# NorESMhub/BLOM

Measured on AMD Instinct MI355X. Metric: simulated-days/sec, higher is better.
Workload: dtype f64; 1 GPU; channel 208x512x53 as 1 tile(s) of 208x512x53 along i, 1 tile per GPU, isopyc_bulkml/remap/geopotential/uc/enscon, ntr=3 (TKE, length-scale slot, ideal age: the reference default build), baclin=900s batrop=18s lstep=50; config 2's step (phy/mod_blom_step.F90:96-253: init_fluxes, tmsmt1, cmnfld2, difest_isobml [the whole routine: diffusivities estimated every step (NorESM defaults incl. rhsctp; the; physics=full, forcing=default, spinup_steps=0

## Files before the change

### blom_amd/csrc/api.hip

```cpp
#include "../../include/blomgpu.h"
#include "blomgpu_internal.h"
#include "pow_libm.h"
#include "sin_libm.h"
#include "atan2_libm.h"
#include <cstring>

static thread_local std::string g_err;

int ctx_fail(blomgpu_ctx *c, const std::string &msg) {
  if (c) c->err = msg;
  g_err = msg;
  return 1;
}

void ctx_drop_graphs(blomgpu_ctx *c) {
  for (auto &g : c->step_graph)
    if (g) { (void)hipGraphExecDestroy(g); g = nullptr; }
  c->steps_warm = 0;
}

void ctx_sync_view(blomgpu_ctx *c) {
  if (!c->dirty) return;
  ctx_drop_graphs(c);
  (void)hipMemcpyAsync(c->d, &c->h, sizeof(DevView), hipMemcpyHostToDevice, c->stream);
// ... 284 lines not shown
  if (s == "tau_decaying_hml") { c->tau_decaying_hml = v; return 0; }
  if (s == "lfmin") { c->lfmin = v; return 0; }
  if (s == "cl") { c->eddtra_cl = v; return 0; }
  if (s == "mstar") { c->mstar = v; return 0; }
  if (s == "nstar") { c->nstar = v; return 0; }
  if (s == "wpup_min") { c->wpup_min = v; return 0; }
  if (s == "mlbl_max_ratio") { c->mlbl_max_ratio = v; return 0; }
  if (s == "ale_stab_fac_limit") { c->ale_stab_fac_limit = v; return 0; }
  if (s == "ale_dpvar_fac") { c->ale_dpvar_fac = v; return 0; }
  if (s == "ale_smooth_diff_max") { c->ale_smooth_diff_max = v; return 0; }
  if (s == "ale_dpmin_interior") { c->ale_dpmin_interior = v * 9806.; return 0; }
  return ctx_fail(c, "blomgpu_set_real: unknown option " + s);
}

int blomgpu_get_real(blomgpu_ctx *c, const char *name, double *v) {
  Params &P = c->h.P;
  std::string s(name);
#define R(nm) if (s == #nm) { *v = P.nm; return 0; }
  R(baclin) R(batrop) R(delt1) R(dlt) R(pref) R(wbaro)
#undef R
  if (s == "area") { *v = c->area; return 0; }
  if (s == "bdml_logc") { *v = c->bdml_logc; return 0; }
  if (s == "barotp_block_mode") { *v = bt_block_mode(c); return 0; }
  if (s == "graph_steps") { *v = c->graph_steps; return 0; }
  if (s == "graph_failures") { *v = c->graph_failures; return 0; }
  if (s == "mxlayr_maxitr_entrain" || s == "mxlayr_maxitr_detrain") {
    *v = 0.;
    if (!c->err_dev) return 0;
    const int w = s == "mxlayr_maxitr_detrain" ? 5 : 6;
    int n = 0;
    HIPCHK(c, hipStreamSynchronize(c->stream));
    HIPCHK(c, hipMemcpy(&n, c->err_dev + w, sizeof(int), hipMemcpyDeviceToHost));
    HIPCHK(c, hipMemset(c->err_dev + w, 0, sizeof(int)));
    *v = n;
    return 0;
  }
  return ctx_fail(c, "blomgpu_get_real: unknown option " + s);
}

int blomgpu_set_int(blomgpu_ctx *c, const char *name, int v) {
  std::string s(name);
  if (c && s == "timing") { c->timing = v != 0; return 0; }
  if (c) ctx_drop_graphs(c);
  Params &P = c->h.P;
#define R(nm) if (s == #nm) { P.nm = v; c->dirty = true; return 0; }
  if (s == "nstep") { P.nstep = v; return 0; }
// ... 676 lines not shown
```

### blom_amd/csrc/blomgpu_internal.h

```cpp
#pragma once
#include <hip/hip_runtime.h>
#include <cstdint>
#include <string>
#include <unordered_map>
#include <vector>
#include "exp_libm.h"

#define NBDY 4

#ifdef BLOM_HOSTEMU
#define WAIT_VMCNT0() ((void)0)
#else
#define WAIT_VMCNT0() asm volatile("s_waitcnt vmcnt(0)" ::: "memory")
#endif

#define BLOM_REAL_FIELDS(X)                                                              \
                                                                          \
  X(u, 2 * K) X(v, 2 * K) X(dp, 2 * K) X(dpu, 2 * K) X(dpv, 2 * K) X(temp, 2 * K)        \
  X(saln, 2 * K) X(sigma, 2 * K) X(uflx, 2 * K) X(vflx, 2 * K) X(utflx, 2 * K)           \
  X(vtflx, 2 * K) X(usflx, 2 * K) X(vsflx, 2 * K)                                        \
  X(p, K + 1) X(pu, K + 1) X(pv, K + 1) X(phi, K + 1) X(cau, K) X(cav, K)                \
  X(ubflxs, 3) X(vbflxs, 3) X(ub, 2) X(vb, 2) X(pb, 2) X(pbu, 2) X(pbv, 2)               \
  X(ubflxs_p, 2) X(vbflxs_p, 2) X(pb_p, 1) X(pbu_p, 1) X(pbv_p, 1) X(ubcors_p, 1)        \
  X(vbcors_p, 1) X(sealv, 1)                                                             \
// ... 206 lines not shown
  int tmsmt_fold = 1;
  bool pbcor1_handed_over = false;
  int steps_warm = 0;
  long long graph_steps = 0;
  int graph_failures = 0;
  int pgf_uv_pair = 0;
  int scan_reassoc = 0;
  hipStream_t side3 = nullptr;
  hipEvent_t ev_side3[2] = {nullptr, nullptr};
  int mom_aw_split = 0;
  int mom_aw_key = -1, mom_aw_n[2] = {0, 0};
  int *mom_aw_dev = nullptr;
  int mom_force_aw = 0;
  int convec_nsingle = 2;
  int cmn_nslope_nb = 4;
  int pgf_reuse = 0;
  int pgf_uv_ring = 7;
  int pgf_copy_fused = 1;
  int eddtra_frozen = 0;
  int check_period = 8;
  bool csdiag = false;
  bool bt_restart = true;
  unsigned bt_epoch = 0;
  int remap_fold = 0;
  int remap_nfirst = 4;
  bool remap_handed_over = false;
  int ale_method = 102, ale_upper_bndr_ord = 6, ale_lower_bndr_ord = 4, ale_tracer_limiting = 203, ale_velocity_limiting = 203;
  bool ale_tracer_pc_upper = true, ale_tracer_pc_lower = false, ale_velocity_pc_upper = true, ale_velocity_pc_lower = false;
  bool ale_density_pc_upper = false, ale_density_pc_lower = false;
  int ale_regrid_method = 2, ale_k_range_plevel = 1;
  double ale_regrid_nudge_ts = 86400., ale_stab_fac_limit = .75, ale_dpvar_fac = .75, ale_smooth_diff_max = 50000.;
  int ale_dktzu = 4, ale_dktzl = 2;
  double ale_dpmin_interior = .1 * 9806.;
  double rm0 = 1.2, rm5 = 0., niwgf = 0., niwbf = .35, niwlf = .5;
  std::string mlrttp = "constant";
  double trxday = 0., srxday = 0., trxdpt = 1., srxdpt = 1., trxlim = 1.5, srxlim = .5, sref = 34.65, area = 0., xmi = 0.;
  int lmi[5] = {11, 12, 1, 2, 3};
  bool aptflx = false, apsflx = false, ditflx = false, disflx = false, srxbal = false;
  int ntda = 0;
  bool full_physics = false;
  double swamxd = 200., brine_mlbase_frac = 0.;
  void *ale = nullptr;
  double *ale_plevel = nullptr;
  int mlrmth = 1;
  double eddtra_ce = .06, tau_mlr = 86400., tau_growing_hbl = 300., tau_decaying_hbl = 86400., tau_growing_hml = 3600.,
         tau_decaying_hml = 259200., lfmin = 5.e3, mlbl_max_ratio = 3., eddtra_cl = .25, mstar = .5, nstar = .066, wpup_min = 1.e-3;
  bool fluxes_lean = false;
// ... 107 lines not shown
int st_mxlayr_tail(blomgpu_ctx *, int nn, int k1n);
int ctx_err_words(blomgpu_ctx *);
int ctx_check_errors(blomgpu_ctx *);
int st_kfpla_halo(blomgpu_ctx *, int n);
int st_cmnfld1(blomgpu_ctx *, int m, int n, int mm, int nn, int k1m, int k1n);
int st_cmnfld2(blomgpu_ctx *, int m, int n, int mm, int nn, int k1m, int k1n);
int diapfl_column3_launch(blomgpu_ctx *, int n, int nn, int *errflag);
#define R_BASE(ntr) (8 + 3 * (ntr))
#define R_DP(ntr) (R_BASE(ntr) + 0)
#define R_T(ntr) (R_BASE(ntr) + 1)
#define R_S(ntr) (R_BASE(ntr) + 2)
#define R_TR(ntr, nt) (R_BASE(ntr) + 3 + (nt))
int st_ale_vdifft(blomgpu_ctx *, int m, int n, int mm, int nn, int k1m, int k1n);
int st_ale_vdiffm(blomgpu_ctx *, int m, int n, int mm, int nn, int k1m, int k1n);
int st_ale_forcing(blomgpu_ctx *, int m, int n, int mm, int nn, int k1m, int k1n);
int st_cmnfld_bfsqi_ale(blomgpu_ctx *, int m, int n, int mm, int nn, int k1m, int k1n);
int st_ale_regrid_remap(blomgpu_ctx *, int m, int n, int mm, int nn, int k1m, int k1n);
void ale_free(blomgpu_ctx *);
int ale_check_deferred(blomgpu_ctx *);
int st_mxlayr(blomgpu_ctx *, int m, int n, int mm, int nn, int k1m, int k1n);
int st_mom_pupv(blomgpu_ctx *, int off, int lo, int hi);
int st_convec_velocity(blomgpu_ctx *, int nn);
int launch_dpudpv(blomgpu_ctx *, int off, int flags);
int remap_tile_launch(blomgpu_ctx *, int n, int mm, int nn, int tsel, bool fold);
int pbcor_tile_launch(blomgpu_ctx *, int which, int m, int offc, int offf, int from_remap);
int launch_pscan(blomgpu_ctx *, int off, int lo, int hi_off);
int st_xctilr(blomgpu_ctx *, double *base, int l1, int ld, int mh, int nh, int itype);
int st_xctilr_arctic_multi(blomgpu_ctx *, int nf, double *const *ptrs, const int *nlevs, const int *mhs, const int *nhs,
                           const int *itypes);
int st_xctilr_multi(blomgpu_ctx *, int nf, double *const *ptrs, const int *nlevs, int mh, int nh, const int *itypes);
int st_crc(blomgpu_ctx *, const double *base, int nlev, int itype, unsigned *crc);
int st_crc_strips(blomgpu_ctx *, double *base, int nlev, int itype, unsigned *out, int cap, int *l0, int *ns);
int ctx_locate_ptr(const blomgpu_ctx *, const double *p, size_t *offset);
int rccl_xctilr(blomgpu_ctx *, double *base, int nlev, int mhl, int nhl);
int rccl_barotp_replicated(blomgpu_ctx *, int m, int n, int mm, int nn, int k1m, int k1n);
blomgpu_ctx *bt_global_ctx(const blomgpu_ctx *);
struct RcclLanded {
  const double *from_west = nullptr, *from_east = nullptr;
  int has_w = 0, has_e = 0, per = 0, mhl = 0, nhl = 0, nlev = 0;
  double *send_west = nullptr, *send_east = nullptr;
  int prepacked = 0;
};
int rccl_xctilr_multi_ex(blomgpu_ctx *, double *const *fields, int nf, int nlev, int mhl, int nhl, RcclLanded *landed);
int rccl_xctilr_multi(blomgpu_ctx *, double *const *fields, int nf, int nlev, int mhl, int nhl);

__device__ inline void xcd_block(unsigned &bx, unsigned &by) {
  const unsigned gx = gridDim.x, n = gx * gridDim.y;
// ... 26 lines not shown
```

### blom_amd/csrc/stage_advect.hip

```cpp
#include "remap_common.h"

#define THREAD_IJ(V)                                                       \
  unsigned bx_, by_;                                                       \
  xcd_block(bx_, by_);                                                     \
  const int t_ = bx_ * blockDim.x + threadIdx.x;                           \
  (void)by_;                                                               \
  if (t_ >= (V).nplane) return;                                            \
  const int i = t_ % (V).ni - (NBDY - 1), j = t_ / (V).ni - (NBDY - 1);    \
  const size_t c = t_

__global__ void k_adv_flux_area(const DevView *__restrict__ Vp, int m, int mm, int nn) {
  const DevView &V = *Vp;
  THREAD_IJ(V);
  if (j < 1 || j > V.jj || i < 1 || i > V.ii) return;
  const int k = by_;
  const size_t np = V.nplane, okm = c + (size_t)(k + mm) * np, okn = c + (size_t)(k + nn) * np;
  const size_t om = c + (size_t)(m - 1) * np;
  const double delt1 = V.P.delt1, dlt = V.P.dlt;
  if (V.m[I_iu][c]) {
    const double dtdl = delt1 * V.f[F_scuy][c];
    const double ca_tmp = V.f[F_u][okm] * dtdl + V.f[F_ubflxs_p][om] * dlt / V.f[F_pbu][om] +
                          (V.f[F_umfltd][okm] + V.f[F_umflsm][okm]) / fmax2(ONEMM, V.f[F_dpu][okn]);
    const double um = V.f[F_umax][c];
    V.f[F_cau][c + (size_t)k * np] = fmax2(-um * dtdl, fmin2(um * dtdl, ca_tmp));
// ... 104 lines not shown
    }
    if (int rc = st_xctilr(c, h.f[F_dp] + (size_t)(k1n - 1) * np, 1, h.kk, 1, 1, 1)) return rc;
    if (int rc = st_xctilr(c, h.f[F_temp] + (size_t)(k1n - 1) * np, 1, h.kk, 1, 1, 1)) return rc;
    if (int rc = st_xctilr(c, h.f[F_saln] + (size_t)(k1n - 1) * np, 1, h.kk, 1, 1, 1)) return rc;
    for (int nt = 0; nt < h.ntr; nt++)
      if (int rc = st_xctilr(c, h.f[F_trc] + ((size_t)(k1n - 1) + (size_t)nt * 2 * h.kk) * np, 1, h.kk, 1, 1, 1)) return rc;
    return 0;
  }
  hipLaunchKernelGGL(k_adv_pbmin, plane_grid(h), dim3(256), 0, c->stream, c->d);
  std::vector<double *> ptrs = {h.f[F_cau], h.f[F_cav]};
  std::vector<int> nl = {h.kk, h.kk}, it = {13, 14};
  for (int nt = 0; nt < h.ntr; nt++) {
    if (trc_skip_adv(h.P, nt + 1)) continue;
    ptrs.push_back(h.f[F_trc] + ((size_t)(k1n - 1) + (size_t)nt * 2 * h.kk) * np);
    nl.push_back(h.kk);
    it.push_back(1);
  }
  const int nf = (int)ptrs.size();
  auto halo_all = [&]() -> int {
    for (int f = 0; f < nf; f += 16)
      if (int rc = st_xctilr_multi(c, nf - f < 16 ? nf - f : 16, ptrs.data() + f, nl.data() + f, 3, 3, it.data() + f)) return rc;
    return 0;
  };
  const bool fold = c->in_sequence && c->remap_fold;
  const int mmlean = !fold && c->in_sequence && c->fluxes_zeroed && c->lean_fluxes ? mm : -1;
  const bool ovl = c->tiling.rccl && c->xstream && c->halo_overlap && !c->timing;
  if (ovl) {
    HIPCHK(c, hipEventRecord(c->ev_fork, c->stream));
    HIPCHK(c, hipStreamWaitEvent(c->xstream, c->ev_fork, 0));
    c->halo_stream = c->xstream;
    const int rc = halo_all();
    c->halo_stream = nullptr;
    if (rc) return rc;
    HIPCHK(c, hipEventRecord(c->ev_join, c->xstream));
    if (int rc2 = remap_tile_launch(c, n, mm, nn, 1, fold)) return rc2;
    HIPCHK(c, hipStreamWaitEvent(c->stream, c->ev_join, 0));
    if (int rc2 = remap_tile_launch(c, n, mm, nn, 2, fold)) return rc2;
    if (!fold) hipLaunchKernelGGL(k_remap_update, plane_grid(h, h.kk), dim3(256), 0, c->stream, c->d, nn, mmlean);
  } else {
    if (int rc = halo_all()) return rc;
    TimeScope ts(c, "remap");
    if (int rc = remap_tile_launch(c, n, mm, nn, 0, fold)) return rc;
    if (!fold) hipLaunchKernelGGL(k_remap_update, plane_grid(h, h.kk), dim3(256), 0, c->stream, c->d, nn, mmlean);
  }
  c->remap_handed_over = fold;
  HIPCHK(c, hipGetLastError());
  return 0;
}
```

### blom_amd/csrc/stage_remap_tile.hip

```cpp
#include "remap_common.h"

#ifndef RT_TH
#define RT_TH 8
#define RT_NT 512
#endif
#define RT_TW 32
#define RT_GW (RT_TW + 2)
#define RT_GN (RT_GW * (RT_TH + 2))
#define RT_SW (RT_TW + 4)
#define RT_SN (RT_SW * (RT_TH + 4))
#define RT_NB 4
#define RT_NSC(ntr) (4 + (ntr))
#define RT_NG(ntr) (10 + 3 * (ntr))
#define RT_G_DPT(ntr) (8 + 3 * (ntr))
#define RT_G_PUP(ntr) (9 + 3 * (ntr))

#define MP(m) ((m) & 1)
#define MU(m) (((m) >> 1) & 1)
#define MV(m) (((m) >> 2) & 1)

static_assert(RT_NT >= RT_SN && RT_NT == 2 * RT_TW * RT_TH, "thread count of k_remap_tile");

#ifdef BLOM_HOSTEMU
#define hmax8 max8
#define hmin8 min8
#define hmax2 fmax2
#define hmin2 fmin2
#else
#define hmax2 hw_max
#define hmin2 hw_min
__device__ inline double hw_max(double a, double b) { double r; asm("v_max_f64 %0, %1, %2" : "=v"(r) : "v"(a), "v"(b)); return r; }
__device__ inline double hw_min(double a, double b) { double r; asm("v_min_f64 %0, %1, %2" : "=v"(r) : "v"(a), "v"(b)); return r; }
__device__ inline double hmax8(double a, double b, double c, double d, double e, double f, double g, double h) {
  return hw_max(hw_max(hw_max(a, b), hw_max(c, d)), hw_max(hw_max(e, f), hw_max(g, h)));
// ... 38 lines not shown
struct AdvList {
  int idx[64];
};
template <bool MORE>
__device__ inline void add_contrib_t(const double *g, int ntr, int x, double pbface, double a, double ax, double ay, double axx,
                                     double ayy, double axy, Acc &A, PolyRec *rec, const int slot) {
  const double dpt = g[RT_G_DPT(ntr) * RT_GN + x];
  const double pup = g[RT_G_PUP(ntr) * RT_GN + x];
  const double dl = fmin2(dpt, fmax2(0., pbface - pup));
  const double dx = g[G_DX * RT_GN + x], dy = g[G_DY * RT_GN + x];
  const double fd = a * dl + ax * dx + ay * dy;
  A.fd = A.fd + fd;
  const double qx = ax * dl + axx * dx + axy * dy;
  const double qy = ay * dl + axy * dx + ayy * dy;
  A.ft = A.ft + fd * g[G_TD * RT_GN + x] + qx * g[G_TX * RT_GN + x] + qy * g[G_TY * RT_GN + x];
  A.fs = A.fs + fd * g[G_SD * RT_GN + x] + qx * g[G_SX * RT_GN + x] + qy * g[G_SY * RT_GN + x];
#pragma unroll
  for (int nt = 0; nt < MAXTR; nt++)
    if (nt < ntr)
      A.ftr[nt] = A.ftr[nt] + fd * g[G_TRD(nt) * RT_GN + x] + qx * g[G_TRX(nt) * RT_GN + x] + qy * g[G_TRY(nt) * RT_GN + x];
  if (MORE) { rec[slot].fd = fd; rec[slot].qx = qx; rec[slot].qy = qy; rec[slot].x = x; }
}

template <bool MORE, bool FOLD>
__global__ void __launch_bounds__(RT_NT, 4) k_remap_tile(const DevView *__restrict__ Vp, int n, int mm, int nn, int ntx, int nadv_all, int nfirst, AdvList L, int tsel KPROF_ARGS) {
  const DevView &V = *Vp;
  const int nadv = nfirst;
  const int base = 1;
  HIP_DYNAMIC_SHARED(double, lds)
  unsigned bx_, by_;
  xcd_block(bx_, by_);
  const int k = by_, ni = V.ni, nj = V.nj, ntr = V.ntr, t = threadIdx.x;
  constexpr int STX = FOLD ? RT_TW - 1 : RT_TW, STY = FOLD ? RT_TH - 1 : RT_TH;
  const int x0 = (bx_ % ntx) * STX, y0 = (bx_ / ntx) * STY;
  const bool zero_old = (tsel & 4) != 0;
  const bool lean = (tsel & 8) != 0;
  tsel &= 3;
  if (tsel) {
    const int jlast = V.jj + NBDY - 1 - ((V.nreg == 2 && V.j0 + V.jj == V.jtdm) ? 1 : 0);
    const bool inner = x0 - 2 >= NBDY && x0 + RT_TW + 1 <= V.ii + NBDY - 1 && y0 - 2 >= NBDY && y0 + RT_TH + 1 <= jlast;
    if (inner != (tsel == 1)) return;
  }
  const size_t np = V.nplane, ok = (size_t)k * np, okn = (size_t)(k + nn) * np, okm = (size_t)(k + mm) * np;
  [[maybe_unused]] const bool kp_on = t == 0 && k == 10;
  if (kp_on) KPROF_MARK(bx_, 0);
  double *const sc = lds;
  double *const gr = lds;
  double *const cuv = lds + RT_NG(nadv) * RT_GN;
  int *const mpl = (int *)(cuv + 2 * RT_GN);
  double *const m2s = (double *)(mpl + RT_SN);
  gci_t mpk = V.m[I_mpack];
  gcd_t scp2 = V.f[F_scp2], scp2i = V.f[F_scp2i];

  double sv[4 + MAXTR];
  int sm;
  size_t cs_keep = 0;
  {
    gcd_t f_dp = V.f[F_dp] + okn, f_p = V.f[F_p] + (size_t)(k + 1) * np, f_t = V.f[F_temp] + okn;
    gcd_t f_s = V.f[F_saln] + okn, f_tr = V.f[F_trc] + okn;
    const int xs = x0 - 2 + t % RT_SW, ys = y0 - 2 + t / RT_SW;
    const bool in = t < RT_SN && xs >= 0 && xs < ni && ys >= 0 && ys < nj;
    const size_t cs = in ? (size_t)ys * ni + xs : 0;
    sm = in ? mpk[cs] : 0;
    sv[0] = f_dp[cs]; sv[1] = f_p[cs]; sv[2] = f_t[cs]; sv[3] = f_s[cs];
#pragma unroll
    for (int a = 0; a < MAXTR; a++) sv[4 + a] = a < nadv ? f_tr[cs + (size_t)L.idx[a] * 2 * V.kk * np] : 0.;
    cs_keep = cs;
  }
  int gx, gy;
  if (t < RT_TW * RT_TH) { gx = t % RT_TW + 1; gy = t / RT_TW + 1; }
  else {
    const int r = t - RT_TW * RT_TH;
    if (r < RT_GW) { gx = r; gy = 0; }
// ... 11 lines not shown
    const bool inplane = gthread && x >= 0 && x < ni && y >= 0 && y < nj;
    const int i = x - (NBDY - 1), j = y - (NBDY - 1);
    const int xc = x < 1 ? 1 : (x > ni - 1 ? ni - 1 : x), yc = y < 1 ? 1 : (y > nj - 1 ? nj - 1 : y);
    const size_t c = (size_t)yc * ni + xc;
    cau_q = V.f[F_cau][c + ok];
    cav_q = V.f[F_cav][c + ok];
    s2_q = scp2[c];
    s2i_q = scp2i[c];
    pm = WK2(V, 0)[c];
    gpoint = inplane && j >= -1 && j <= V.jj + 2 && i >= -1 && i <= V.ii + 2;
  }
  const bool uface = t < RT_TW * RT_TH;
  const int ft = t % (RT_TW * RT_TH);
  const int fq = (ft / RT_TW + 1) * RT_GW + ft % RT_TW + 1;
  const int fx = x0 + ft % RT_TW, fy = y0 + ft / RT_TW;
  const bool fin = fx >= 1 && fx < ni - 1 && fy >= 1 && fy < nj - 1;
  const size_t fc = fin ? (size_t)fy * ni + fx : (size_t)ni + 1;
  const int fi = fx - (NBDY - 1), fj = fy - (NBDY - 1);
  const double caf = (uface ? V.f[F_cau] : V.f[F_cav])[fc + ok];
  const double pbf = (uface ? V.f[F_pbu] : V.f[F_pbv])[fc + (size_t)(n - 1) * np];
  gd_t const o_f = (uface ? V.f[F_uflx] : V.f[F_vflx]) + fc + okm;
  gd_t const o_ft = (uface ? V.f[F_utflx] : V.f[F_vtflx]) + fc + okm;
  gd_t const o_fs = (uface ? V.f[F_usflx] : V.f[F_vsflx]) + fc + okm;
  const bool own = !FOLD || (ft % RT_TW < RT_TW - 1 && ft / RT_TW < RT_TH - 1);
  const bool rd_old = uface && !zero_old && own;
  const double f_o = rd_old ? *o_f : 0., ft_o = rd_old ? *o_ft : 0., fs_o = rd_old ? *o_fs : 0.;

  if (t < RT_SN) {
    mpl[t] = sm;
#pragma unroll
    for (int s = 0; s < 4 + MAXTR; s++)
      if (s < 4 + nadv) sc[s * RT_SN + t] = sv[s];
  }
  if (gthread) { cuv[q] = cau_q; cuv[RT_GN + q] = cav_q; m2s[q] = s2_q; m2s[RT_GN + q] = s2i_q; }
  __syncthreads();
  if (kp_on) KPROF_MARK(bx_, 1);

  double gv[10 + 3 * MAXTR];
#pragma unroll
  for (int s = 0; s < 10 + 3 * MAXTR; s++) gv[s] = 0.;
  double cuc = 0., cvc = 0.;
  const int mpc = gthread ? mpl[sidx] : 0;
  gpoint = gpoint && MP(mpc);
  TNbr nb;
  nb.w = nb.e = nb.s = nb.n = nb.sw = nb.se = nb.nw = nb.ne = 0;
  double k_dxi = 0., k_dyi = 0., k_xd = 0., k_yd = 0.;
  if (gpoint) {
    const int a = MU(mpc), b = MU(mpl[sidx + 1]), d = MV(mpc), e = MV(mpl[sidx + RT_SW]);
    nb.w = sidx - a;
// ... 68 lines not shown
    for (int s = 0; s < 8 + 3 * MAXTR; s++)
      if (s < 8 + 3 * nadv) gr[s * RT_GN + q] = gv[s];
    gr[RT_G_DPT(nadv) * RT_GN + q] = gv[8 + 3 * MAXTR];
    gr[RT_G_PUP(nadv) * RT_GN + q] = gv[9 + 3 * MAXTR];
    cuv[q] = cuc;
    cuv[RT_GN + q] = cvc;
  }
  __syncthreads();
  if (kp_on) KPROF_MARK(bx_, 2);
  if (!MORE && !FOLD && !fin) return;

  const int mpf = fin ? mpl[(ft / RT_TW + 2) * RT_SW + ft % RT_TW + 2] : 0;
  const bool fmask = uface ? MU(mpf) : MV(mpf);
  const bool in_f = uface ? (fj >= 0 && fj <= V.jj + 1 && fi >= 0 && fi <= V.ii + 2) : (fj >= 0 && fj <= V.jj + 2 && fi >= 0 && fi <= V.ii + 1);
  if (!MORE && !FOLD && !in_f) return;
  const bool do_face = fin && in_f;
  PolyRec rec[3];
#pragma unroll
  for (int z = 0; z < 3; z++) { rec[z].fd = 0.; rec[z].qx = 0.; rec[z].qy = 0.; rec[z].x = fq; }
  Acc A;
  A.fd = 0.; A.ft = 0.; A.fs = 0.;
#pragma unroll
  for (int nt = 0; nt < MAXTR; nt++) A.ftr[nt] = 0.;
  if (do_face) {
  const int f_along = uface ? 1 : RT_GW, f_across = uface ? RT_GW : 1;
  const double cf = fmask ? (caf > 0. ? caf * m2s[RT_GN + fq - f_along] : caf * m2s[RT_GN + fq]) : 0.;
  if (fmask) {
    const double cuc0 = cuv[fq], cvc0 = cuv[RT_GN + fq];
    const bool near = cf > 0.;
    const double sh = near ? .5 : -.5;
    const int fb = near ? fq - f_along : fq;
    const double s2_c = m2s[fb], s2_m = m2s[fb - f_across], s2_p = m2s[fb + f_across];
    const double s2i_m = m2s[RT_GN + fb - f_across], s2i_p = m2s[RT_GN + fb + f_across];
    double a, ax, ay, axx, ayy, axy, x2, y2, x4, y4;
    if (uface) {
      const double cuc1 = cuv[fq + RT_GW], cvc1 = cuv[RT_GN + fq + RT_GW];
      const double ym = -.5 * (cvc0 + cvc1);
      const double xm = ((ym + .5) * cuc0 - (ym - .5) * cuc1 - 2. * cf) / (1. + cvc0 - cvc1);
      const int ic = near ? fq - 1 : fq;
      if (cvc0 > 0.) {
        const double xc0 = (xm * cvc0 - cuc0 * (ym + .5)) / (cvc0 + ym + .5);
        const double xc1 = xc0 * s2_c * s2i_m;
        x4 = xc0 + sh;
        y4 = -.5;
        triint(s2_m, xc1 + sh, .5, -cuc0 + sh, -cvc0 + .5, sh, .5, a, ax, ay, axx, ayy, axy);
        add_contrib_t<MORE>(gr, nadv, ic - RT_GW, pbf, a, ax, ay, axx, ayy, axy, A, rec, 0);
      } else {
        x4 = -cuc0 + sh;
        y4 = -cvc0 - .5;
      }
      if (cvc1 < 0.) {
        const double xc0 = (xm * cvc1 - cuc1 * (ym - .5)) / (cvc1 + ym - .5);
        const double xc1 = xc0 * s2_c * s2i_p;
        x2 = xc0 + sh;
        y2 = .5;
        triint(s2_p, xc1 + sh, -.5, sh, -.5, -cuc1 + sh, -cvc1 - .5, a, ax, ay, axx, ayy, axy);
        add_contrib_t<MORE>(gr, nadv, ic + RT_GW, pbf, a, ax, ay, axx, ayy, axy, A, rec, 1);
      } else {
        x2 = -cuc1 + sh;
        y2 = -cvc1 + .5;
      }
      penint(s2_c, sh, .5, x2, y2, xm + sh, ym, x4, y4, sh, -.5, a, ax, ay, axx, ayy, axy);
      add_contrib_t<MORE>(gr, nadv, ic, pbf, a, ax, ay, axx, ayy, axy, A, rec, 2);
      if (base && own) {
        *o_f = f_o + A.fd;
        *o_ft = ft_o + A.ft;
        *o_fs = fs_o + A.fs;
      }
    } else {
      const double cuc1 = cuv[fq + 1], cvc1 = cuv[RT_GN + fq + 1];
      const double xm = -.5 * (cuc0 + cuc1);
      const double ym = ((xm + .5) * cvc0 - (xm - .5) * cvc1 - 2. * cf) / (1. + cuc0 - cuc1);
      const int jc = near ? fq - RT_GW : fq;
      if (cuc0 > 0.) {
        const double yc0 = (ym * cuc0 - cvc0 * (xm + .5)) / (cuc0 + xm + .5);
        const double yc1 = yc0 * s2_c * s2i_m;
        x2 = -.5;
        y2 = yc0 + sh;
        triint(s2_m, .5, yc1 + sh, .5, sh, -cuc0 + .5, -cvc0 + sh, a, ax, ay, axx, ayy, axy);
        add_contrib_t<MORE>(gr, nadv, jc - 1, pbf, a, ax, ay, axx, ayy, axy, A, rec, 0);
      } else {
        x2 = -cuc0 - .5;
        y2 = -cvc0 + sh;
      }
      if (cuc1 < 0.) {
        const double yc0 = (ym * cuc1 - cvc1 * (xm - .5)) / (cuc1 + xm - .5);
        const double yc1 = yc0 * s2_c * s2i_p;
        x4 = .5;
        y4 = yc0 + sh;
        triint(s2_p, -.5, yc1 + sh, -cuc1 - .5, -cvc1 + sh, -.5, sh, a, ax, ay, axx, ayy, axy);
        add_contrib_t<MORE>(gr, nadv, jc + 1, pbf, a, ax, ay, axx, ayy, axy, A, rec, 1);
      } else {
        x4 = -cuc1 + .5;
        y4 = -cvc1 + sh;
      }
      penint(s2_c, -.5, sh, x2, y2, xm, ym + sh, x4, y4, .5, sh, a, ax, ay, axx, ayy, axy);
      add_contrib_t<MORE>(gr, nadv, jc, pbf, a, ax, ay, axx, ayy, axy, A, rec, 2);
      if (base && own) {
        *o_f = A.fd;
        *o_ft = A.ft;
        *o_fs = A.fs;
      }
    }
  }
  const int off = uface ? 0 : 1;
  if (!FOLD) {
    if (base && !lean) {
      WK(V, W_FDU(ntr) + off)[fc + ok] = A.fd;
      WK(V, W_FTU(ntr) + off)[fc + ok] = A.ft;
      WK(V, W_FSU(ntr) + off)[fc + ok] = A.fs;
    }
#pragma unroll
    for (int nt = 0; nt < MAXTR; nt++)
      if (nt < nadv) WK(V, W_FTRU(ntr, L.idx[nt]) + off)[fc + ok] = A.ftr[nt];
  }
  }
  const int cx = fx - (NBDY - 1), cy = fy - (NBDY - 1);
  const bool upd = FOLD && uface && own && fin && cy >= 0 && cy <= V.jj + 1 && cx >= 0 && cx <= V.ii + 1 && MP(mpf);
  double q_dp = 0., dpn = 1.;
  double *const fl = lds;
  if (FOLD) {
    __syncthreads();
    fl[t] = A.fd; fl[RT_NT + t] = A.ft; fl[2 * RT_NT + t] = A.fs;
#pragma unroll
    for (int nt = 0; nt < MAXTR; nt++)
      if (nt < nadv) fl[(3 + nt) * RT_NT + t] = A.ftr[nt];
    __syncthreads();
    if (upd) {
      const int te = t + 1, ts = RT_TW * RT_TH + t, tn = ts + RT_TW;
      const double s2i = m2s[RT_GN + fq];
      q_dp = fmax2(0., V.f[F_dp][fc + okn]) + DPEPS;
      dpn = q_dp - (fl[te] - fl[t] + fl[tn] - fl[ts]) * s2i;
      const double told = V.f[F_temp][fc + okn], sold = V.f[F_saln][fc + okn];
      WK(V, R_T(ntr))[fc + ok] = (q_dp * told - (fl[RT_NT + te] - fl[RT_NT + t] + fl[RT_NT + tn] - fl[RT_NT + ts]) * s2i) / dpn;
      WK(V, R_S(ntr))[fc + ok] = (q_dp * sold - (fl[2 * RT_NT + te] - fl[2 * RT_NT + t] + fl[2 * RT_NT + tn] - fl[2 * RT_NT + ts]) * s2i) / dpn;
#pragma unroll
      for (int nt = 0; nt < MAXTR; nt++)
        if (nt < nadv) {
          const double *f = fl + (3 + nt) * RT_NT;
          const double xold = V.f[F_trc][fc + okn + (size_t)L.idx[nt] * 2 * V.kk * np];
          WK(V, R_TR(ntr, L.idx[nt]))[fc + ok] = (q_dp * xold - (f[te] - f[t] + f[tn] - f[ts]) * s2i) / dpn;
        }
      WK(V, R_DP(ntr))[fc + ok] = fmax2(0., dpn - DPEPS);
    }
  }
  if (!MORE) {
    if (kp_on) KPROF_MARK(bx_, 3);
    return;
  }
  gcd_t f_tr = V.f[F_trc] + okn;
  const int off2 = uface ? 0 : 1;
  if constexpr (!FOLD) {
    double *const bs = lds, *const bg = lds + RT_NB * RT_SN;
    double tv[RT_NB], gb[3 * RT_NB];
#pragma unroll
    for (int a = 0; a < 3 * RT_NB; a++) gb[a] = 0.;
    auto fetch = [&](int b0) {
#pragma unroll
      for (int a = 0; a < RT_NB; a++)
        tv[a] = (b0 + a < nadv_all && t < RT_SN) ? f_tr[cs_keep + (size_t)L.idx[b0 + a < 64 ? b0 + a : 0] * 2 * V.kk * np] : 0.;
    };
    fetch(nadv);
    __syncthreads();
    if (kp_on) KPROF_MARK(bx_, 3);
// ... 112 lines not shown
    i = t % w - 2;
  } else {
    t -= 6 * w;
    if (t >= 6 * jj) return;
    j = t / 6 + 1;
    const int q = t % 6;
    i = q < 3 ? q - 2 : ii + 1 + (q - 3);
  }
  const size_t c = IDX(V, i, j);
  if (!V.m[I_ip][c]) return;
  const int k = blockIdx.y, ntr = V.ntr;
  const size_t np = V.nplane, ok = (size_t)k * np, okn = (size_t)(k + nn) * np;
  if (j < 0 || j > jj + 1 || i < 0 || i > ii + 1) {
    V.f[F_dp][c + okn] = fmax2(0., V.f[F_dp][c + okn]) + DPEPS;
    return;
  }
  V.f[F_dp][c + okn] = WK(V, R_DP(ntr))[c + ok];
  V.f[F_temp][c + okn] = WK(V, R_T(ntr))[c + ok];
  V.f[F_saln][c + okn] = WK(V, R_S(ntr))[c + ok];
  for (int a = 0; a < nadv_all; a++)
    V.f[F_trc][c + okn + (size_t)L.idx[a] * 2 * V.kk * np] = WK(V, R_TR(ntr, L.idx[a]))[c + ok];
}

int remap_tile_launch(blomgpu_ctx *c, int n, int mm, int nn, int tsel, bool fold) {
  const bool zeroed = c->in_sequence && c->fluxes_zeroed;
  if (tsel == 0 || tsel == 2) c->fluxes_zeroed = false;
  if (zeroed) tsel |= 4;
  if (zeroed && !fold && c->lean_fluxes) tsel |= 8;
  if (c->fluxes_lean && !(tsel & 8)) return ctx_fail(c, "remap: the flux arrays were zeroed on their ring only (lean init_fluxes) but the storing tile path is not taken");
  if (tsel == (tsel | 8) && ((tsel & 3) == 0 || (tsel & 3) == 2)) c->fluxes_lean = false;
  const DevView &h = c->h;
  const int stx = fold ? RT_TW - 1 : RT_TW, sty = fold ? RT_TH - 1 : RT_TH;
  const int ntx = (h.ni + stx - 1) / stx, nty = (h.nj + sty - 1) / sty;
  static_assert(RT_NSC(MAXTR) * RT_SN <= RT_NG(MAXTR) * RT_GN, "the scalars must fit under the gradient slots");
  if (h.ntr > 255) return ctx_fail(c, "remap: tracer indices are packed in 8 bits");
  if (h.ntr > 0 && W_FTRV(h.ntr, h.ntr - 1) >= h.nwk) return ctx_fail(c, "remap: work space too small for this many tracers");
  AdvList L;
  int nadv = 0;
  for (int nt = 0; nt < h.ntr; nt++)
    if (!trc_skip_adv(h.P, nt + 1)) {
      if (nadv == 64) return ctx_fail(c, "remap: more than 64 advected tracers");
      L.idx[nadv++] = nt;
    }
  for (int a = nadv; a < 64; a++) L.idx[a] = 0;
  int nfirst = nadv < MAXTR ? nadv : MAXTR;
  if (nadv > MAXTR && !fold) nfirst = c->remap_nfirst < MAXTR ? (c->remap_nfirst > 0 ? c->remap_nfirst : 0) : MAXTR;
  size_t lds = sizeof(double) * (RT_NG(nfirst) * RT_GN + 2 * RT_GN) + sizeof(int) * RT_SN + sizeof(double) * 2 * RT_GN;
  if (nadv > MAXTR && !fold && lds < sizeof(double) * RT_NB * (RT_SN + 3 * RT_GN)) lds = sizeof(double) * RT_NB * (RT_SN + 3 * RT_GN);
  const dim3 grid(ntx * nty, h.kk);
  if (fold) {
    {
      TimeScope tk(c, "k_remap_tile");
      if (nadv > MAXTR) hipLaunchKernelGGL((k_remap_tile<true, true>), grid, dim3(RT_NT), lds, c->stream, c->d, n, mm, nn, ntx, nadv, nfirst, L, tsel KPROF_PASS(9));
      else hipLaunchKernelGGL((k_remap_tile<false, true>), grid, dim3(RT_NT), lds, c->stream, c->d, n, mm, nn, ntx, nadv, nfirst, L, tsel KPROF_PASS(9));
    }
    if ((tsel & 3) != 1)
      hipLaunchKernelGGL(k_remap_ring, dim3((6 * (h.ii + 6) + 6 * h.jj + 63) / 64, h.kk), dim3(64), 0, c->stream, c->d, nn, nadv, L);
  } else {
    TimeScope tk(c, "k_remap_tile");
    if (nadv > MAXTR) hipLaunchKernelGGL((k_remap_tile<true, false>), grid, dim3(RT_NT), lds, c->stream, c->d, n, mm, nn, ntx, nadv, nfirst, L, tsel KPROF_PASS(9));
    else hipLaunchKernelGGL((k_remap_tile<false, false>), grid, dim3(RT_NT), lds, c->stream, c->d, n, mm, nn, ntx, nadv, nfirst, L, tsel KPROF_PASS(9));
  }
  return 0;
}
```

### blom_amd/csrc/stage_simple.hip

```cpp
#include "blomgpu_internal.h"

#define PLANE_IJ(V)                                                        \
  unsigned bx_, by_;                                                       \
  xcd_block(bx_, by_);                                                     \
  const int t_ = bx_ * blockDim.x + threadIdx.x;                           \
  (void)by_;                                                               \
  if (t_ >= (V).nplane) return;                                            \
  const int i = t_ % (V).ni - (NBDY - 1), j = t_ / (V).ni - (NBDY - 1);    \
  const size_t c = t_;                                                     \
  (void)i; (void)j; (void)c

__global__ void k_init_fluxes(const DevView *__restrict__ Vp, int mm) {
  const DevView &V = *Vp;
  PLANE_IJ(V);
  if (j < 0 || j > V.jj + 2 || i < 0 || i > V.ii + 2) return;
  const size_t o = c + (size_t)(by_ + mm) * V.nplane;
  if (V.m[I_iu][c]) { V.f[F_uflx][o] = 0.; V.f[F_utflx][o] = 0.; V.f[F_usflx][o] = 0.; }
  if (V.m[I_iv][c]) { V.f[F_vflx][o] = 0.; V.f[F_vtflx][o] = 0.; V.f[F_vsflx][o] = 0.; }
}

__global__ void k_init_fluxes_ring(const DevView *__restrict__ Vp, int mm) {
  const DevView &V = *Vp;
  const int t = blockIdx.x * blockDim.x + threadIdx.x, k = blockIdx.y;
  const int nu = V.ii + 3, nv = V.jj + 3;
  const size_t off = (size_t)(k + mm) * V.nplane;
  if (t < nu) {
    const size_t c = IDX(V, t, V.jj + 2);
    if (V.m[I_iu][c]) { V.f[F_uflx][c + off] = 0.; V.f[F_utflx][c + off] = 0.; V.f[F_usflx][c + off] = 0.; }
  } else if (t < nu + nv) {
    const size_t c = IDX(V, V.ii + 2, t - nu);
    if (V.m[I_iv][c]) { V.f[F_vflx][c + off] = 0.; V.f[F_vtflx][c + off] = 0.; V.f[F_vsflx][c + off] = 0.; }
  }
}

int st_init_fluxes(blomgpu_ctx *c, int m, int n, int mm, int nn, int k1m, int k1n) {
  (void)m; (void)n; (void)nn; (void)k1m; (void)k1n;
  const DevView &h = c->h;
  TimeScope ts(c, "init_fluxes");
  if (c->in_sequence && c->lean_fluxes && h.P.advmth == 0 && h.P.vcoord_tag == 1 && !c->remap_fold) {
    hipLaunchKernelGGL(k_init_fluxes_ring, dim3((h.ii + h.jj + 6 + 63) / 64, h.kk), dim3(64), 0, c->stream, c->d, mm);
    HIPCHK(c, hipGetLastError());
    c->fluxes_zeroed = true;
    c->fluxes_lean = true;
    return 0;
  }
  hipLaunchKernelGGL(k_init_fluxes, plane_grid(c->h, c->h.kk), dim3(256), 0, c->stream, c->d, mm);
  HIPCHK(c, hipGetLastError());
  c->fluxes_zeroed = c->in_sequence;
  c->fluxes_lean = false;
  return 0;
}

__global__ void k_tmsmt1(const DevView *__restrict__ Vp, int off, int is_initms) {
  const DevView &V = *Vp;
  PLANE_IJ(V);
  if (j < 1 || j > V.jj || i < 1 || i > V.ii) return;
  const int k = by_;
  const size_t ok = c + (size_t)k * V.nplane, okn = c + (size_t)(k + off) * V.nplane;
  if (V.m[I_ip][c]) {
    if (!is_initms) V.f[F_dpold][okn] = V.f[F_dp][okn];
    V.f[F_told][ok] = V.f[F_temp][okn];
    V.f[F_sold][ok] = V.f[F_saln][okn];
// ... 326 lines not shown
```

Baseline: 1.657 simulated-days/sec.

## Add non-overlapping fold mode to remap tile with recomputed edge fluxes

Adds a new FOLD=2 layout for the remap tile kernel and makes it the default. Tiles no longer overlap by one cell as in FOLD=1. Instead, dedicated threads recompute the east and north boundary face fluxes into shared memory, so each tile can fuse the tracer/layer-thickness update without redundant tiles. Old tracer values and dp' are fetched early from the gradient slot rather than reread, and the lean ring-only flux zeroing remains allowed. The cost is extra LDS, extra per-tile flux work on the edge threads, and more register pressure in a complex kernel.

```diff
diff --git a/blom_amd/csrc/api.hip b/blom_amd/csrc/api.hip
--- a/blom_amd/csrc/api.hip
+++ b/blom_amd/csrc/api.hip
@@ -330,6 +330,7 @@
   if (s == "area") { *v = c->area; return 0; }
   if (s == "bdml_logc") { *v = c->bdml_logc; return 0; }
   if (s == "barotp_block_mode") { *v = bt_block_mode(c); return 0; }
+  if (s == "remap_layout") { *v = remap_layout(c, true); return 0; }
   if (s == "graph_steps") { *v = c->graph_steps; return 0; }
   if (s == "graph_failures") { *v = c->graph_failures; return 0; }
   if (s == "mxlayr_maxitr_entrain" || s == "mxlayr_maxitr_detrain") {
diff --git a/blom_amd/csrc/blomgpu_internal.h b/blom_amd/csrc/blomgpu_internal.h
--- a/blom_amd/csrc/blomgpu_internal.h
+++ b/blom_amd/csrc/blomgpu_internal.h
@@ -252,7 +252,7 @@
   bool csdiag = false;
   bool bt_restart = true;
   unsigned bt_epoch = 0;
-  int remap_fold = 0;
+  int remap_fold = 2;
   int remap_nfirst = 4;
   bool remap_handed_over = false;
   int ale_method = 102, ale_upper_bndr_ord = 6, ale_lower_bndr_ord = 4, ale_tracer_limiting = 203, ale_velocity_limiting = 203;
@@ -406,7 +406,8 @@
 int st_mom_pupv(blomgpu_ctx *, int off, int lo, int hi);
 int st_convec_velocity(blomgpu_ctx *, int nn);
 int launch_dpudpv(blomgpu_ctx *, int off, int flags);
-int remap_tile_launch(blomgpu_ctx *, int n, int mm, int nn, int tsel, bool fold);
+int remap_tile_launch(blomgpu_ctx *, int n, int mm, int nn, int tsel, int fold);
+int remap_layout(const blomgpu_ctx *, bool in_step = false);
 int pbcor_tile_launch(blomgpu_ctx *, int which, int m, int offc, int offf, int from_remap);
 int launch_pscan(blomgpu_ctx *, int off, int lo, int hi_off);
 int st_xctilr(blomgpu_ctx *, double *base, int l1, int ld, int mh, int nh, int itype);
diff --git a/blom_amd/csrc/stage_advect.hip b/blom_amd/csrc/stage_advect.hip
--- a/blom_amd/csrc/stage_advect.hip
+++ b/blom_amd/csrc/stage_advect.hip
@@ -150,7 +150,7 @@
       if (int rc = st_xctilr_multi(c, nf - f < 16 ? nf - f : 16, ptrs.data() + f, nl.data() + f, 3, 3, it.data() + f)) return rc;
     return 0;
   };
-  const bool fold = c->in_sequence && c->remap_fold;
+  const int fold = remap_layout(c);
   const int mmlean = !fold && c->in_sequence && c->fluxes_zeroed && c->lean_fluxes ? mm : -1;
   const bool ovl = c->tiling.rccl && c->xstream && c->halo_overlap && !c->timing;
   if (ovl) {
@@ -171,7 +171,7 @@
     if (int rc = remap_tile_launch(c, n, mm, nn, 0, fold)) return rc;
     if (!fold) hipLaunchKernelGGL(k_remap_update, plane_grid(h, h.kk), dim3(256), 0, c->stream, c->d, nn, mmlean);
   }
-  c->remap_handed_over = fold;
+  c->remap_handed_over = fold != 0;
   HIPCHK(c, hipGetLastError());
   return 0;
 }
diff --git a/blom_amd/csrc/stage_remap_tile.hip b/blom_amd/csrc/stage_remap_tile.hip
--- a/blom_amd/csrc/stage_remap_tile.hip
+++ b/blom_amd/csrc/stage_remap_tile.hip
@@ -10,6 +10,9 @@
 #define RT_SW (RT_TW + 4)
 #define RT_SN (RT_SW * (RT_TH + 4))
 #define RT_NB 4
+#define RT_NX (RT_TW + RT_TH)
+#define RT_XU (3 * 64)
+#define RT_XV (7 * 64)
 #define RT_NSC(ntr) (4 + (ntr))
 #define RT_NG(ntr) (10 + 3 * (ntr))
 #define RT_G_DPT(ntr) (8 + 3 * (ntr))
@@ -94,8 +97,9 @@
   if (MORE) { rec[slot].fd = fd; rec[slot].qx = qx; rec[slot].qy = qy; rec[slot].x = x; }
 }
 
-template <bool MORE, bool FOLD>
+template <bool MORE, int FOLD>
 __global__ void __launch_bounds__(RT_NT, 4) k_remap_tile(const DevView *__restrict__ Vp, int n, int mm, int nn, int ntx, int nadv_all, int nfirst, AdvList L, int tsel KPROF_ARGS) {
+  static_assert(!(MORE && FOLD == 2), "k_remap_tile: FOLD 2 has no batch loop");
   const DevView &V = *Vp;
   const int nadv = nfirst;
   const int base = 1;
@@ -103,7 +107,7 @@
   unsigned bx_, by_;
   xcd_block(bx_, by_);
   const int k = by_, ni = V.ni, nj = V.nj, ntr = V.ntr, t = threadIdx.x;
-  constexpr int STX = FOLD ? RT_TW - 1 : RT_TW, STY = FOLD ? RT_TH - 1 : RT_TH;
+  constexpr int STX = FOLD == 1 ? RT_TW - 1 : RT_TW, STY = FOLD == 1 ? RT_TH - 1 : RT_TH;
   const int x0 = (bx_ % ntx) * STX, y0 = (bx_ / ntx) * STY;
   const bool zero_old = (tsel & 4) != 0;
   const bool lean = (tsel & 8) != 0;
@@ -121,6 +125,8 @@
   double *const cuv = lds + RT_NG(nadv) * RT_GN;
   int *const mpl = (int *)(cuv + 2 * RT_GN);
   double *const m2s = (double *)(mpl + RT_SN);
+  double *const xd = m2s + 2 * RT_GN;
+  double *const xfl = xd + 2 * RT_NX;
   gci_t mpk = V.m[I_mpack];
   gcd_t scp2 = V.f[F_scp2], scp2i = V.f[F_scp2i];
 
@@ -178,9 +184,27 @@
   gd_t const o_f = (uface ? V.f[F_uflx] : V.f[F_vflx]) + fc + okm;
   gd_t const o_ft = (uface ? V.f[F_utflx] : V.f[F_vtflx]) + fc + okm;
   gd_t const o_fs = (uface ? V.f[F_usflx] : V.f[F_vsflx]) + fc + okm;
-  const bool own = !FOLD || (ft % RT_TW < RT_TW - 1 && ft / RT_TW < RT_TH - 1);
+  const bool own = FOLD != 1 || (ft % RT_TW < RT_TW - 1 && ft / RT_TW < RT_TH - 1);
   const bool rd_old = uface && !zero_old && own;
   const double f_o = rd_old ? *o_f : 0., ft_o = rd_old ? *o_ft : 0., fs_o = rd_old ? *o_fs : 0.;
+  auto xface = [&](int &xe, int &xlx, int &xly, int &xfx, int &xfy, bool &xfin) {
+    xe = FOLD != 2 ? -1 : (t >= RT_XU && t < RT_XU + RT_TH) ? t - RT_XU : (t >= RT_XV && t < RT_XV + RT_TW) ? RT_TH + t - RT_XV : -1;
+    xlx = uface ? RT_TW : xe - RT_TH;
+    xly = uface ? xe : RT_TH;
+    xfx = x0 + xlx;
+    xfy = y0 + xly;
+    xfin = xe >= 0 && xfx >= 1 && xfx < ni - 1 && xfy >= 1 && xfy < nj - 1;
+  };
+  if (FOLD == 2) {
+    int xe, xlx, xly, xfx, xfy;
+    bool xfin;
+    xface(xe, xlx, xly, xfx, xfy, xfin);
+    if (xe >= 0) {
+      const size_t xc = xfin ? (size_t)xfy * ni + xfx : (size_t)ni + 1;
+      xd[xe] = (uface ? V.f[F_cau] : V.f[F_cav])[xc + ok];
+      xd[RT_NX + xe] = (uface ? V.f[F_pbu] : V.f[F_pbv])[xc + (size_t)(n - 1) * np];
+    }
+  }
 
   if (t < RT_SN) {
     mpl[t] = sm;
@@ -295,10 +319,9 @@
   A.fd = 0.; A.ft = 0.; A.fs = 0.;
 #pragma unroll
   for (int nt = 0; nt < MAXTR; nt++) A.ftr[nt] = 0.;
-  if (do_face) {
-  const int f_along = uface ? 1 : RT_GW, f_across = uface ? RT_GW : 1;
-  const double cf = fmask ? (caf > 0. ? caf * m2s[RT_GN + fq - f_along] : caf * m2s[RT_GN + fq]) : 0.;
-  if (fmask) {
+  auto face_flux = [&](const int fq, const double caf, const double pbf, Acc &A, PolyRec *rec) {
+    const int f_along = uface ? 1 : RT_GW, f_across = uface ? RT_GW : 1;
+    const double cf = caf > 0. ? caf * m2s[RT_GN + fq - f_along] : caf * m2s[RT_GN + fq];
     const double cuc0 = cuv[fq], cvc0 = cuv[RT_GN + fq];
     const bool near = cf > 0.;
     const double sh = near ? .5 : -.5;
@@ -335,11 +358,6 @@
       }
       penint(s2_c, sh, .5, x2, y2, xm + sh, ym, x4, y4, sh, -.5, a, ax, ay, axx, ayy, axy);
       add_contrib_t<MORE>(gr, nadv, ic, pbf, a, ax, ay, axx, ayy, axy, A, rec, 2);
-      if (base && own) {
-        *o_f = f_o + A.fd;
-        *o_ft = ft_o + A.ft;
-        *o_fs = fs_o + A.fs;
-      }
     } else {
       const double cuc1 = cuv[fq + 1], cvc1 = cuv[RT_GN + fq + 1];
       const double xm = -.5 * (cuc0 + cuc1);
@@ -369,7 +387,36 @@
       }
       penint(s2_c, -.5, sh, x2, y2, xm, ym + sh, x4, y4, .5, sh, a, ax, ay, axx, ayy, axy);
       add_contrib_t<MORE>(gr, nadv, jc, pbf, a, ax, ay, axx, ayy, axy, A, rec, 2);
-      if (base && own) {
+    }
+  };
+  int xe = -1, xlx, xly, xfx, xfy;
+  bool xfin;
+  if (FOLD == 2) xface(xe, xlx, xly, xfx, xfy, xfin);
+  if (FOLD == 2 && xe >= 0) {
+    const int xq = (xly + 1) * RT_GW + xlx + 1;
+    const int xfi = xfx - (NBDY - 1), xfj = xfy - (NBDY - 1);
+    const int xmp = xfin ? mpl[(xly + 2) * RT_SW + xlx + 2] : 0;
+    const bool xin = uface ? (xfj >= 0 && xfj <= V.jj + 1 && xfi >= 0 && xfi <= V.ii + 2) : (xfj >= 0 && xfj <= V.jj + 2 && xfi >= 0 && xfi <= V.ii + 1);
+    Acc X;
+    X.fd = 0.; X.ft = 0.; X.fs = 0.;
+#pragma unroll
+    for (int nt = 0; nt < MAXTR; nt++) X.ftr[nt] = 0.;
+    PolyRec xrec[3];
+    if (xfin && xin && (uface ? MU(xmp) : MV(xmp))) face_flux(xq, xd[xe], xd[RT_NX + xe], X, xrec);
+    xfl[xe] = X.fd; xfl[RT_NX + xe] = X.ft; xfl[2 * RT_NX + xe] = X.fs;
+#pragma unroll
+    for (int nt = 0; nt < MAXTR; nt++)
+      if (nt < nadv) xfl[(3 + nt) * RT_NX + xe] = X.ftr[nt];
+  }
+  if (do_face) {
+  if (fmask) {
+    face_flux(fq, caf, pbf, A, rec);
+    if (base && own) {
+      if (uface) {
+        *o_f = f_o + A.fd;
+        *o_ft = ft_o + A.ft;
+        *o_fs = fs_o + A.fs;
+      } else {
         *o_f = A.fd;
         *o_ft = A.ft;
         *o_fs = A.fs;
@@ -392,6 +439,15 @@
   const bool upd = FOLD && uface && own && fin && cy >= 0 && cy <= V.jj + 1 && cx >= 0 && cx <= V.ii + 1 && MP(mpf);
   double q_dp = 0., dpn = 1.;
   double *const fl = lds;
+  double o_t = 0., o_s = 0., o_tr[MAXTR];
+  if (FOLD == 2 && upd) {
+    o_t = V.f[F_temp][fc + okn];
+    o_s = V.f[F_saln][fc + okn];
+#pragma unroll
+    for (int nt = 0; nt < MAXTR; nt++) o_tr[nt] = nt < nadv ? V.f[F_trc][fc + okn + (size_t)L.idx[nt] * 2 * V.kk * np] : 0.;
+    q_dp = gr[RT_G_DPT(nadv) * RT_GN + fq];
+  }
+  static_assert(3 * RT_NT <= RT_G_DPT(0) * RT_GN && (3 + MAXTR) * RT_NT <= RT_G_DPT(MAXTR) * RT_GN, "the flux slots lie below the dp' slot");
   if (FOLD) {
     __syncthreads();
     fl[t] = A.fd; fl[RT_NT + t] = A.ft; fl[2 * RT_NT + t] = A.fs;
@@ -400,19 +456,24 @@
       if (nt < nadv) fl[(3 + nt) * RT_NT + t] = A.ftr[nt];
     __syncthreads();
     if (upd) {
-      const int te = t + 1, ts = RT_TW * RT_TH + t, tn = ts + RT_TW;
+      const bool xeast = FOLD == 2 && ft % RT_TW == RT_TW - 1, xnorth = FOLD == 2 && ft / RT_TW == RT_TH - 1;
+      const int xb = (int)(xfl - lds);
+      const int te = xeast ? xb + ft / RT_TW : t + 1, se = xeast ? RT_NX : RT_NT;
+      const int ts = RT_TW * RT_TH + t;
+      const int tn = xnorth ? xb + RT_TH + ft % RT_TW : ts + RT_TW, sn = xnorth ? RT_NX : RT_NT;
       const double s2i = m2s[RT_GN + fq];
-      q_dp = fmax2(0., V.f[F_dp][fc + okn]) + DPEPS;
+      if (FOLD == 1) q_dp = fmax2(0., V.f[F_dp][fc + okn]) + DPEPS;
       dpn = q_dp - (fl[te] - fl[t] + fl[tn] - fl[ts]) * s2i;
-      const double told = V.f[F_temp][fc + okn], sold = V.f[F_saln][fc + okn];
-      WK(V, R_T(ntr))[fc + ok] = (q_dp * told - (fl[RT_NT + te] - fl[RT_NT + t] + fl[RT_NT + tn] - fl[RT_NT + ts]) * s2i) / dpn;
-      WK(V, R_S(ntr))[fc + ok] = (q_dp * sold - (fl[2 * RT_NT + te] - fl[2 * RT_NT + t] + fl[2 * RT_NT + tn] - fl[2 * RT_NT + ts]) * s2i) / dpn;
+      const double told = FOLD == 2 ? o_t : V.f[F_temp][fc + okn], sold = FOLD == 2 ? o_s : V.f[F_saln][fc + okn];
+      WK(V, R_T(ntr))[fc + ok] = (q_dp * told - (fl[se + te] - fl[RT_NT + t] + fl[sn + tn] - fl[RT_NT + ts]) * s2i) / dpn;
+      WK(V, R_S(ntr))[fc + ok] = (q_dp * sold - (fl[2 * se + te] - fl[2 * RT_NT + t] + fl[2 * sn + tn] - fl[2 * RT_NT + ts]) * s2i) / dpn;
 #pragma unroll
       for (int nt = 0; nt < MAXTR; nt++)
         if (nt < nadv) {
-          const double *f = fl + (3 + nt) * RT_NT;
-          const double xold = V.f[F_trc][fc + okn + (size_t)L.idx[nt] * 2 * V.kk * np];
-          WK(V, R_TR(ntr, L.idx[nt]))[fc + ok] = (q_dp * xold - (f[te] - f[t] + f[tn] - f[ts]) * s2i) / dpn;
+          const int s = 3 + nt;
+          const double *f = fl + s * RT_NT;
+          const double xold = FOLD == 2 ? o_tr[nt] : V.f[F_trc][fc + okn + (size_t)L.idx[nt] * 2 * V.kk * np];
+          WK(V, R_TR(ntr, L.idx[nt]))[fc + ok] = (q_dp * xold - (fl[s * se + te] - f[t] + fl[s * sn + tn] - f[ts]) * s2i) / dpn;
         }
       WK(V, R_DP(ntr))[fc + ok] = fmax2(0., dpn - DPEPS);
     }
@@ -571,44 +632,60 @@
     V.f[F_trc][c + okn + (size_t)L.idx[a] * 2 * V.kk * np] = WK(V, R_TR(ntr, L.idx[a]))[c + ok];
 }
 
-int remap_tile_launch(blomgpu_ctx *c, int n, int mm, int nn, int tsel, bool fold) {
+static int adv_list(const DevView &h, AdvList &L) {
+  int nadv = 0;
+  for (int nt = 0; nt < h.ntr; nt++)
+    if (!trc_skip_adv(h.P, nt + 1)) {
+      if (nadv < 64) L.idx[nadv] = nt;
+      nadv++;
+    }
+  for (int a = nadv; a < 64; a++) L.idx[a] = 0;
+  return nadv;
+}
+
+int remap_layout(const blomgpu_ctx *c, bool in_step) {
+  if (!(in_step || c->in_sequence) || c->remap_fold <= 0) return 0;
+  if (c->remap_fold == 1) return 1;
+  AdvList L;
+  return adv_list(c->h, L) > MAXTR ? 0 : 2;
+}
+
+int remap_tile_launch(blomgpu_ctx *c, int n, int mm, int nn, int tsel, int fold) {
   const bool zeroed = c->in_sequence && c->fluxes_zeroed;
   if (tsel == 0 || tsel == 2) c->fluxes_zeroed = false;
   if (zeroed) tsel |= 4;
-  if (zeroed && !fold && c->lean_fluxes) tsel |= 8;
+  if (zeroed && fold != 1 && c->lean_fluxes) tsel |= 8;
   if (c->fluxes_lean && !(tsel & 8)) return ctx_fail(c, "remap: the flux arrays were zeroed on their ring only (lean init_fluxes) but the storing tile path is not taken");
   if (tsel == (tsel | 8) && ((tsel & 3) == 0 || (tsel & 3) == 2)) c->fluxes_lean = false;
   const DevView &h = c->h;
-  const int stx = fold ? RT_TW - 1 : RT_TW, sty = fold ? RT_TH - 1 : RT_TH;
+  const int stx = fold == 1 ? RT_TW - 1 : RT_TW, sty = fold == 1 ? RT_TH - 1 : RT_TH;
   const int ntx = (h.ni + stx - 1) / stx, nty = (h.nj + sty - 1) / sty;
   static_assert(RT_NSC(MAXTR) * RT_SN <= RT_NG(MAXTR) * RT_GN, "the scalars must fit under the gradient slots");
   if (h.ntr > 255) return ctx_fail(c, "remap: tracer indices are packed in 8 bits");
   if (h.ntr > 0 && W_FTRV(h.ntr, h.ntr - 1) >= h.nwk) return ctx_fail(c, "remap: work space too small for this many tracers");
   AdvList L;
-  int nadv = 0;
-  for (int nt = 0; nt < h.ntr; nt++)
-    if (!trc_skip_adv(h.P, nt + 1)) {
-      if (nadv == 64) return ctx_fail(c, "remap: more than 64 advected tracers");
-      L.idx[nadv++] = nt;
-    }
-  for (int a = nadv; a < 64; a++) L.idx[a] = 0;
+  const int nadv = adv_list(h, L);
+  if (nadv > 64) return ctx_fail(c, "remap: more than 64 advected tracers");
+  if (fold == 2 && nadv > MAXTR) return ctx_fail(c, "remap: FOLD 2 takes at most MAXTR advected tracers");
   int nfirst = nadv < MAXTR ? nadv : MAXTR;
   if (nadv > MAXTR && !fold) nfirst = c->remap_nfirst < MAXTR ? (c->remap_nfirst > 0 ? c->remap_nfirst : 0) : MAXTR;
   size_t lds = sizeof(double) * (RT_NG(nfirst) * RT_GN + 2 * RT_GN) + sizeof(int) * RT_SN + sizeof(double) * 2 * RT_GN;
   if (nadv > MAXTR && !fold && lds < sizeof(double) * RT_NB * (RT_SN + 3 * RT_GN)) lds = sizeof(double) * RT_NB * (RT_SN + 3 * RT_GN);
+  if (fold == 2) lds += sizeof(double) * (2 + 3 + nfirst) * RT_NX;
   const dim3 grid(ntx * nty, h.kk);
   if (fold) {
     {
       TimeScope tk(c, "k_remap_tile");
-      if (nadv > MAXTR) hipLaunchKernelGGL((k_remap_tile<true, true>), grid, dim3(RT_NT), lds, c->stream, c->d, n, mm, nn, ntx, nadv, nfirst, L, tsel KPROF_PASS(9));
-      else hipLaunchKernelGGL((k_remap_tile<false, true>), grid, dim3(RT_NT), lds, c->stream, c->d, n, mm, nn, ntx, nadv, nfirst, L, tsel KPROF_PASS(9));
+      if (fold == 2) hipLaunchKernelGGL((k_remap_tile<false, 2>), grid, dim3(RT_NT), lds, c->stream, c->d, n, mm, nn, ntx, nadv, nfirst, L, tsel KPROF_PASS(9));
+      else if (nadv > MAXTR) hipLaunchKernelGGL((k_remap_tile<true, 1>), grid, dim3(RT_NT), lds, c->stream, c->d, n, mm, nn, ntx, nadv, nfirst, L, tsel KPROF_PASS(9));
+      else hipLaunchKernelGGL((k_remap_tile<false, 1>), grid, dim3(RT_NT), lds, c->stream, c->d, n, mm, nn, ntx, nadv, nfirst, L, tsel KPROF_PASS(9));
     }
     if ((tsel & 3) != 1)
       hipLaunchKernelGGL(k_remap_ring, dim3((6 * (h.ii + 6) + 6 * h.jj + 63) / 64, h.kk), dim3(64), 0, c->stream, c->d, nn, nadv, L);
   } else {
     TimeScope tk(c, "k_remap_tile");
-    if (nadv > MAXTR) hipLaunchKernelGGL((k_remap_tile<true, false>), grid, dim3(RT_NT), lds, c->stream, c->d, n, mm, nn, ntx, nadv, nfirst, L, tsel KPROF_PASS(9));
-    else hipLaunchKernelGGL((k_remap_tile<false, false>), grid, dim3(RT_NT), lds, c->stream, c->d, n, mm, nn, ntx, nadv, nfirst, L, tsel KPROF_PASS(9));
+    if (nadv > MAXTR) hipLaunchKernelGGL((k_remap_tile<true, 0>), grid, dim3(RT_NT), lds, c->stream, c->d, n, mm, nn, ntx, nadv, nfirst, L, tsel KPROF_PASS(9));
+    else hipLaunchKernelGGL((k_remap_tile<false, 0>), grid, dim3(RT_NT), lds, c->stream, c->d, n, mm, nn, ntx, nadv, nfirst, L, tsel KPROF_PASS(9));
   }
   return 0;
 }
diff --git a/blom_amd/csrc/stage_simple.hip b/blom_amd/csrc/stage_simple.hip
--- a/blom_amd/csrc/stage_simple.hip
+++ b/blom_amd/csrc/stage_simple.hip
@@ -37,7 +37,7 @@
   (void)m; (void)n; (void)nn; (void)k1m; (void)k1n;
   const DevView &h = c->h;
   TimeScope ts(c, "init_fluxes");
-  if (c->in_sequence && c->lean_fluxes && h.P.advmth == 0 && h.P.vcoord_tag == 1 && !c->remap_fold) {
+  if (c->in_sequence && c->lean_fluxes && h.P.advmth == 0 && h.P.vcoord_tag == 1 && remap_layout(c) != 1) {
     hipLaunchKernelGGL(k_init_fluxes_ring, dim3((h.ii + h.jj + 6 + 63) / 64, h.kk), dim3(64), 0, c->stream, c->d, mm);
     HIPCHK(c, hipGetLastError());
     c->fluxes_zeroed = true;
```

New measurement: 1.676 simulated-days/sec, median of 6. 1.01x the previous value.
